# MKimiSH/video-filler

Measured on AMD Instinct MI355X. Metric: netG+netD fwd+bwd images/sec, 128x128 center-mask, higher is better.
Workload: dtype f32

## Files before the change

include/vf_hip.h:

```cpp
#ifndef VF_HIP_H
#define VF_HIP_H
#include <stddef.h>
#include <stdint.h>
#ifdef __cplusplus
extern "C" {
#endif

typedef struct vf_ctx vf_ctx;

enum { VF_ACT_NONE = 0, VF_ACT_LRELU = 1, VF_ACT_RELU = 2, VF_ACT_TANH = 3, VF_ACT_SIGMOID = 4 };

const char* vf_last_error(void);
int vf_version(void);
int vf_ctx_create(vf_ctx** out, int device, void* stream);
int vf_ctx_destroy(vf_ctx* ctx);
int vf_ctx_set_mfma_mode(vf_ctx* ctx, int mode);
int vf_ctx_set_stream(vf_ctx* ctx, void* stream);
int vf_ctx_set_workspace(vf_ctx* ctx, void* ptr, size_t bytes);
size_t vf_workspace_bytes_hint(void);
int vf_stream_synchronize(vf_ctx* ctx);
int vf_malloc(void** out, size_t bytes);
int vf_free(void* ptr);
int vf_memcpy_h2d(vf_ctx* ctx, void* dst, const void* src, size_t bytes);
int vf_memcpy_d2h(vf_ctx* ctx, void* dst, const void* src, size_t bytes);
// ... 154 lines not shown
                   int32_t* status, int32_t* rounds);

int vf_channel_copy(vf_ctx* ctx, const float* src, int Csrc, int c_src, float* dst, int Cdst, int c_dst, int Ccopy,
                    int64_t npix);
int vf_noise_fill(vf_ctx* ctx, float* out, int64_t n, uint64_t seed, const int32_t* counter_dev, uint64_t counter,
                  int normal);

int vf_wgrad_group_begin(vf_ctx* ctx);
int vf_wgrad_group_end(vf_ctx* ctx);
int vf_wgrad_group_abort(vf_ctx* ctx);
int vf_wgrad_group_count(vf_ctx* ctx, int* count);
int vf_wgrad_group_end_partial(vf_ctx* ctx, int count);

int vf_bias_grad_plan(int64_t P, int C, int* cq, int* rows_per_block, int* gx, int* gy);
int vf_bias_grad_multi(vf_ctx* ctx, const void* desc_dev, int n, int blocks1, int blocks2);

typedef struct vf_comm vf_comm;
#define VF_COMM_ID_BYTES 128
int vf_comm_available(void);
int vf_comm_unique_id(void* id128);
int vf_comm_init(vf_comm** out, const void* id128, int world, int rank);
int vf_comm_world(const vf_comm* c);
int vf_comm_rank(const vf_comm* c);
int vf_comm_allreduce_async(vf_comm* c, vf_ctx* ctx, void* buf, int64_t count, int dtype, int op, int* ticket);
int vf_comm_allreduce_avg_async(vf_comm* c, vf_ctx* ctx, float* buf, int64_t n, int* ticket);
int vf_comm_reduce_scatter_avg_async(vf_comm* c, vf_ctx* ctx, float* buf, int64_t shard_count, int* ticket);
int vf_comm_allgather_async(vf_comm* c, vf_ctx* ctx, float* buf, int64_t shard_count, int* ticket);
int vf_comm_broadcast_async(vf_comm* c, vf_ctx* ctx, float* buf, int64_t count, int root, int* ticket);
int vf_comm_wait(vf_comm* c, vf_ctx* ctx, int ticket);
int vf_comm_allreduce_inline(vf_comm* c, vf_ctx* ctx, void* buf, int64_t count, int dtype, int op);
// ... 78 lines not shown
```

video-filler_amd/_lib.py:

```python
import ctypes as C
import os
import re

_HERE = os.path.dirname(os.path.abspath(__file__))
_HEADER = os.path.join(_HERE, "..", "include", "vf_hip.h")

vp, f32, i32, i64, f64, sz, u64 = C.c_void_p, C.c_float, C.c_int, C.c_int64, C.c_double, C.c_size_t, C.c_uint64

SIGNATURES = {
    "vf_last_error": (C.c_char_p, []),
    "vf_version": (i32, []),
    "vf_ctx_create": (i32, [C.POINTER(vp), i32, vp]),
    "vf_ctx_destroy": (i32, [vp]),
    "vf_ctx_set_mfma_mode": (i32, [vp, i32]),
    "vf_ctx_set_stream": (i32, [vp, vp]),
    "vf_ctx_set_workspace": (i32, [vp, vp, sz]),
    "vf_workspace_bytes_hint": (sz, []),
    "vf_stream_synchronize": (i32, [vp]),
    "vf_malloc": (i32, [C.POINTER(vp), sz]),
    "vf_free": (i32, [vp]),
    "vf_memcpy_h2d": (i32, [vp, vp, vp, sz]),
    "vf_memcpy_d2h": (i32, [vp, vp, vp, sz]),
    "vf_zero": (i32, [vp, vp, sz]),
    "vf_zero_segments": (i32, [vp, vp, vp, vp, i32]),
# ... 31 lines not shown
    "vf_bn_fuse_result": (i32, [vp, C.POINTER(i32)]),
    "vf_bn_train_fwd_pre": (i32, [vp, vp, i32] + [vp] * 9 + [i64, i32, i32, f32, f32, i32, f32, vp]),
    "vf_bn_bwd_pre": (i32, [vp, vp, i32] + [vp] * 9 + [i64, i32, i32, f32, vp]),
    "vf_act_fwd": (i32, [vp, vp, vp, i64, i32, f32]),
    "vf_act_bwd": (i32, [vp, vp, vp, vp, i64, i32, f32]),
    "vf_axpby": (i32, [vp, f32, vp, f32, vp, i64]),
    "vf_cmul": (i32, [vp, vp, vp, i64]),
    "vf_scale_shift": (i32, [vp, vp, f32, f32, i64]),
    "vf_masked_compose": (i32, [vp, vp, vp, vp, vp, i64]),
    "vf_conv2d_bwd_data_act": (i32, [vp, vp, vp, vp, vp, i32, f32, i32, i32, i32, i32, i32, i32, i32, i32]),
    "vf_wgrad_group_begin": (i32, [vp]),
    "vf_wgrad_group_end": (i32, [vp]),
    "vf_wgrad_group_abort": (i32, [vp]),
    "vf_bias_grad_plan": (i32, [i64, i32, vp, vp, vp, vp]),
    "vf_bias_grad_multi": (i32, [vp, vp, i32, i32, i32]),
    "vf_center_prepare": (i32, [vp, vp, vp, vp, vp, i32, i32, i32, i32]),
    "vf_clip_prepare": (i32, [vp, vp, vp, vp, vp, vp, i32, i32, i32, i32, i32, i32, i32, f32, i32, i32, vp, vp]),
    "vf_tiles_gather": (i32, [vp, vp, vp, i32, i32, i32, i32, i32, vp]),
    "vf_tiles_scatter": (i32, [vp, vp, vp, i32, i32, i32, i32, i32, vp]),
    "vf_image_scale": (i32, [vp, vp, i32, vp] + [i32] * 6),
    "vf_image_scale_u8": (i32, [vp, vp, vp] + [i32] * 6),
    "vf_image_hook2d": (i32, [vp, vp, i32, vp] + [i32] * 9),
    "vf_image_whole_frames": (i32, [vp, vp, i32, vp] + [i32] * 8 + [vp, f32]),
    "vf_crop_stats": (i32, [vp, vp, vp] + [i32] * 6 + [vp]),
    "vf_jpeg_inspect": (i32, [vp, sz, i32, vp, C.c_char_p, i32]),
    "vf_jpeg_workspace_bytes": (i32, [vp, vp, i32, i32, C.POINTER(sz), C.POINTER(sz)]),
    "vf_jpeg_decode": (i32, [vp, vp, vp, i32, i32, i32, vp, vp, vp, sz, vp, sz, vp, vp]),
    "vf_channel_copy": (i32, [vp, vp, i32, i32, vp, i32, i32, i32, i64]),
    "vf_noise_fill": (i32, [vp, vp, i64, u64, vp, u64, i32]),
    "vf_bce_fwd": (i32, [vp, vp, f32, i32, vp]),
# ... 131 lines not shown
```

video-filler_amd/backend.py:

```python
import ctypes as C
import os

import numpy as np
import torch

from . import _lib

ACT = {"none": 0, "lrelu": 1, "relu": 2, "tanh": 3, "sigmoid": 4}
COLSUM_DESC = [("g", "<u8"), ("gb", "<u8"), ("part", "<u8"), ("P", "<i8"), ("C", "<i4"), ("cq", "<i4"), ("rows_per_block", "<i4"),
               ("gx", "<i4"), ("gy", "<i4"), ("blk1_off", "<i4"), ("blk2_off", "<i4"), ("beta", "<f4")]
WPLANES_DESC = [("w", "<u8"), ("nat", "<u8"), ("tr", "<u8"), ("d0", "<i4"), ("d1", "<i4"), ("gx", "<i4"), ("gz", "<i4"),
                ("blk_off", "<i4"), ("pad", "<i4")]
MFMA_MODES = {"f32": 0, "bf16": 1, "f32_3xbf16": 3}
DEFAULT_MFMA_MODE = "f32_3xbf16"


_COMM_DTYPE = {torch.float32: 0, torch.float64: 1}
_COMM_OP = {"sum": 0, "avg": 1, "max": 2, "min": 3}


class _Range:
    def __init__(self, lib, name):
        self.lib, self.name = lib, name.encode()

# ... 391 lines not shown
    def wgrad_group_abort(self):
        self._c("vf_wgrad_group_abort")

    def wgrad_group_count(self):
        n = C.c_int(0)
        self._c("vf_wgrad_group_count", C.byref(n))
        return n.value

    def wgrad_group_end_partial(self, count):
        self._c("vf_wgrad_group_end_partial", int(count))

    def bias_grad_multi(self, items):
        import numpy as np
        if not items:
            return
        key = tuple((g.data_ptr(), gb.data_ptr(), g.numel(), gb.numel(), float(beta)) for g, gb, beta in items)
        cache = self.__dict__.setdefault("_colsum_plans", {})
        plan = cache.get(key)
        if plan is None:
            desc = np.zeros(len(items), dtype=COLSUM_DESC)
            ws = self.workspace.data_ptr()
            off, b1, b2 = 0, 0, 0
            for i, (g, gb, beta) in enumerate(items):
                Cc = gb.numel()
                P = g.numel() // Cc
                assert Cc % 4 == 0 and g.data_ptr() % 16 == 0 and is_nhwc(g)
                geo = [C.c_int() for _ in range(4)]
                _lib.check(self.lib.vf_bias_grad_plan(P, Cc, *[C.byref(v) for v in geo]))
                cq, rpb, gx, gy = [v.value for v in geo]
                desc[i] = (g.data_ptr(), gb.data_ptr(), ws + off, P, Cc, cq, rpb, gx, gy, b1, b2, beta)
                off += (gx * Cc * 8 + 255) // 256 * 256
                b1 += gx * gy
                b2 += (Cc + 3) // 4
            assert off <= self.workspace.numel(), "workspace too small for the bias-gradient partials"
            dev = torch.from_numpy(desc.view(np.uint8).copy()).to(self.device)
            plan = (dev, len(items), b1, b2)
            cache[key] = plan
        dev, n, b1, b2 = plan
        self._c("vf_bias_grad_multi", _ptr(dev), n, b1, b2)

    def conv2d_bwd_weight(self, x, gy, gw, gb, k, stride, pad, beta, x_planes=None, gy_planes=None):
        B, Cin, H, W = x.shape
        if x_planes is not None and gy_planes is not None:
            self._c("vf_conv2d_bwd_weight_planes", _ptr(x), _ptr(gy), _ptr(x_planes), _ptr(gy_planes), _ptr(gw), _ptr(gb), B, H, W,
                    Cin, gw.shape[0], k, stride, pad, beta)
            return
        self._c("vf_conv2d_bwd_weight", _ptr(x), _ptr(gy), _ptr(gw), _ptr(gb), B, H, W, Cin, gw.shape[0], k, stride,
                pad, beta)

    def deconv2d_fwd(self, x, w, bias, y, k, stride, pad, act="none", slope=0.0):
        B, Cin, H, W = x.shape
        self._c("vf_deconv2d_fwd", _ptr(x), _ptr(w), _ptr(bias), _ptr(y), B, H, W, Cin, w.shape[1], k, stride, pad,
                ACT[act], slope)

# ... 405 lines not shown
```

video-filler_amd/csrc/vf_bn.hip:

```cpp
#include <algorithm>

#include "vf_common.h"

typedef float f32x4 __attribute__((ext_vector_type(4)));
typedef unsigned int u32x2 __attribute__((ext_vector_type(2)));

__device__ __forceinline__ unsigned bn_rne16(float v) {
  const unsigned u = __float_as_uint(v);
  return (u + 0x7FFFu + ((u >> 16) & 1u)) >> 16;
}
__device__ __forceinline__ void bn_store_planes(unsigned short* __restrict__ planes, int64_t pstride, int64_t i, f32x4 v, int npl) {
  if (npl == 1) {
    u32x2 o;
    o[0] = bn_rne16(v[0]) | (bn_rne16(v[1]) << 16);
    o[1] = bn_rne16(v[2]) | (bn_rne16(v[3]) << 16);
    *(u32x2*)(planes + i) = o;
    return;
  }
  float r0 = v[0], r1 = v[1], r2 = v[2], r3 = v[3];
#pragma unroll
  for (int q = 0; q < 3; ++q) {
    const unsigned u0 = __float_as_uint(r0), u1 = __float_as_uint(r1), u2 = __float_as_uint(r2), u3 = __float_as_uint(r3);
    u32x2 o;
    o[0] = __builtin_amdgcn_perm(u1, u0, 0x07060302u);
// ... 665 lines not shown
                       2 * C, sums, (float*)nullptr, (float*)nullptr, (float*)nullptr, (float*)nullptr, 0.0, 0.f, 0.f, (float*)nullptr,
                       0.f, 1);
    VF_LAUNCH_CHECK();
  }
  return bn_bwd_apply_groups(ctx, x, nullptr, g_masked, gx, ggamma, gbeta, gamma, save_mean, save_invstd, sums, npix_per_group,
                             npix_per_group, C, groups, VF_ACT_NONE, 0.f, pbeta, gx_planes);
}

VF_API int vf_bias_grad_plan(int64_t P, int C, int* cq, int* rows_per_block, int* gx, int* gy) {
  VF_REQUIRE(P > 0 && C > 0 && C % 4 == 0, "vf_bias_grad_plan: C must be a positive multiple of 4 (got %d)", C);
  const BnGeom g = bn_geom(P, C, bn_stat_blocks(P, C, 32768));
  *cq = g.cq; *rows_per_block = g.rows_per_block; *gx = g.gx; *gy = g.gy;
  return 0;
}
VF_API int vf_bias_grad_multi(vf_ctx* ctx, const void* desc_dev, int n, int blocks1, int blocks2) {
  VF_REQUIRE(desc_dev != nullptr && n > 0 && blocks1 > 0 && blocks2 > 0, "vf_bias_grad_multi: empty plan");
  VfProf prof(ctx, "bias_grad_multi", 0.0, 0.0);
  hipLaunchKernelGGL(k_colsum4_multi, dim3(blocks1), dim3(256), 0, ctx->stream, (const VfColsumDesc*)desc_dev, n);
  VF_LAUNCH_CHECK();
  hipLaunchKernelGGL(k_reduce_bias_multi, dim3(blocks2), dim3(256), 0, ctx->stream, (const VfColsumDesc*)desc_dev, n);
  VF_LAUNCH_CHECK();
  return 0;
}
```

video-filler_amd/csrc/vf_common.h:

```cpp
#pragma once
#include <hip/hip_runtime.h>
#include <hip/hip_ext.h>

#include <cstdarg>
#include <cstdint>
#include <cstdio>
#include <cstring>

#include "../../include/vf_hip.h"

#define VF_API extern "C" __attribute__((visibility("default")))

struct VfBnSt {
  int mode;
  const float* vec;
  const float* x;
  double* part;
  int rows_per_group;
  int tiles_per_group;
  int zpar;
};

struct vf_ctx {
  int device;
// ... 4 lines not shown
  int mfma_bf16;
  int wg_active;
  void* wg_rec;
  VfBnSt bnf;
  const float* bnf_yact;
  int bnf_act;
  float bnf_slope;
  int bnf_groups, bnf_rows_cap;
  int bnf_result_rows;
  unsigned* act_bits_out;
  int act_bits_written;
  const unsigned* dmask_bits;
  const float* dot_act_y;
  int dot_act;
  float dot_act_slope;
};
void vf_internal_wg_free(vf_ctx* ctx);

unsigned vf_error_seq();
struct VfOneShotScope {
  vf_ctx* c;
  unsigned seq;
  explicit VfOneShotScope(vf_ctx* ctx) : c(ctx), seq(vf_error_seq()) {}
  ~VfOneShotScope() {
    if (!c || vf_error_seq() == seq) return;
    c->bnf.mode = 0;
    c->bnf_result_rows = 0;
    c->act_bits_out = nullptr;
    c->act_bits_written = 0;
    c->dmask_bits = nullptr;
    c->dot_act_y = nullptr;
  }
};

static inline char* vf_ws_ptr(vf_ctx* c) { return (char*)c->ws + c->ws_front; }
static inline size_t vf_ws_avail(vf_ctx* c) { return c->ws_bytes > c->ws_front ? c->ws_bytes - c->ws_front : 0; }

void vf_set_error(const char* fmt, ...);

#define VF_CHECK_HIP(expr)                                                              \
  do {                                                                                  \
    hipError_t _e = (expr);                                                             \
    if (_e != hipSuccess) {                                                             \
      vf_set_error("%s:%d: %s failed: %s", __FILE__, __LINE__, #expr, hipGetErrorString(_e)); \
      return 1;                                                                         \
    }                                                                                   \
// ... 133 lines not shown
```

video-filler_amd/csrc/vf_conv.hip:

```cpp
#include <algorithm>
#include <vector>
#include <cstdlib>

#include "vf_common.h"

typedef float f32x16 __attribute__((ext_vector_type(16)));
typedef float f32x4 __attribute__((ext_vector_type(4)));
typedef unsigned int u32x4 __attribute__((ext_vector_type(4)));
typedef __bf16 bf16x8 __attribute__((ext_vector_type(8)));
typedef __bf16 bf16x4 __attribute__((ext_vector_type(4)));

#define VF_OOB 0x80000000u
__device__ __forceinline__ __amdgpu_buffer_rsrc_t vf_rsrc(const void* p, unsigned bytes) {
  return __builtin_amdgcn_make_buffer_rsrc(const_cast<void*>(p), 0, bytes, 0x00020000);
}
__device__ __forceinline__ f32x4 vf_bload4(__amdgpu_buffer_rsrc_t r, unsigned byte_off) {
  return __builtin_bit_cast(f32x4, __builtin_amdgcn_raw_buffer_load_b128(r, byte_off, 0, 0));
}
__device__ __forceinline__ float vf_bload1(__amdgpu_buffer_rsrc_t r, unsigned byte_off) {
  return __builtin_bit_cast(float, __builtin_amdgcn_raw_buffer_load_b32(r, byte_off, 0, 0));
}

template <int LD>
__device__ __forceinline__ bf16x8 vf_tr_frag(const __bf16* tile, int col0, int k0, int lane) {
// ... 764 lines not shown
}

struct WGrad {
  const float* U;
  const float* V;
  float* dW;
  float* slab;
  unsigned u_bytes, v_bytes;
  int P, lgMh, lgMw;
  int Nu, Cv, Hv, Wv;
  int stride, pad;
  int ntaps;
  int gx, gy, gz;
  int ksplit, nk;
  float beta;
};

template <int BM, bool VU, bool VV, int BF = 0>
__device__ __forceinline__ void wgrad_body(const WGrad& p, const int block_id) {
  constexpr int BN = 128, BK = BF ? 32 : 16;
  constexpr int LDU = BM + 4, LDV = BN + 4;
  constexpr int WN = BM == 128 ? 64 : 32;
  constexpr int NT = WN / 32;
  constexpr int WAVES_N = BN / WN;
  constexpr int U_CH = (BK * BM / 4) / 256;
  constexpr int V_CH = (BK * BN / 4) / 256;
  constexpr int U_SZ = BK * LDU, V_SZ = BK * LDV;
  constexpr int LDMU = BM + 32, LDMV = BN + 32;
  constexpr int UH_SZ = BK * LDMU, VH_SZ = BK * LDMV;
  constexpr int NP = BF > 0 ? BF : 1;
// ... 16 lines not shown
  int v_dy[4], v_dx[4], v_c[4];
  bool v_okc[4];
#pragma unroll
  for (int j = 0; j < 4; ++j) {
    const int col = j0 + 4 * cq + j;
    v_okc[j] = col < Ncols;
    const int tap = v_okc[j] ? col / p.Cv : 0;
    v_c[j] = v_okc[j] ? col - tap * p.Cv : 0;
    v_dy[j] = (tap >> 2) - p.pad;
    v_dx[j] = (tap & 3) - p.pad;
  }
  const int uq = tid % (BM / 4), ukk = tid / (BM / 4);
  const int un = n0 + 4 * uq;

  f32x4 ru[U_CH], rv[V_CH];
  const __amdgpu_buffer_rsrc_t rsU = vf_rsrc(p.U, p.u_bytes), rsV = vf_rsrc(p.V, p.v_bytes);

  auto load_piece = [&](int kt, int pc, bool live) {
    if (pc < U_CH) {
      const int i = pc;
      const int pp = kt * BK + ukk + i * (1024 / BM);
      const bool okp = live && pp < p.P;
      if constexpr (VU) {
        ru[i] = vf_bload4(rsU, (okp && un < p.Nu) ? 4u * (unsigned)(pp * p.Nu + un) : VF_OOB);
      } else {
        f32x4 v;
#pragma unroll
        for (int j = 0; j < 4; ++j) {
          v[j] = vf_bload1(rsU, (okp && un + j < p.Nu) ? 4u * (unsigned)(pp * p.Nu + un + j) : VF_OOB);
        }
// ... 10 lines not shown
        const bool ok = okp && v_okc[0] && (unsigned)iy < (unsigned)p.Hv && (unsigned)ix < (unsigned)p.Wv;
        rv[i] = vf_bload4(rsV, ok ? 4u * (unsigned)(boff + (iy * p.Wv + ix) * p.Cv + v_c[0]) : VF_OOB);
      } else {
        f32x4 v;
#pragma unroll
        for (int j = 0; j < 4; ++j) {
          const int iy = my * p.stride + v_dy[j], ix = mx * p.stride + v_dx[j];
          const bool ok = okp && v_okc[j] && (unsigned)iy < (unsigned)p.Hv && (unsigned)ix < (unsigned)p.Wv;
          v[j] = vf_bload1(rsV, ok ? 4u * (unsigned)(boff + (iy * p.Wv + ix) * p.Cv + v_c[j]) : VF_OOB);
        }
        rv[i] = v;
      }
    }
  };
  auto store_piece = [&](int buf, int pc) {
    if constexpr (BF) {
      __bf16* base = (__bf16*)smem + buf * (NP * PL_SZ);
      f32x4 v;
      int off;
      if (pc < U_CH) {
        v = ru[pc];
        off = (ukk + pc * (1024 / BM)) * LDMU + 4 * uq;
      } else {
        const int i = pc - U_CH;
        v = rv[i];
        off = UH_SZ + ((tid >> 5) + 8 * i) * LDMV + 4 * cq;
      }
      if constexpr (NP == 3) {
        const VfPlanes3 s3 = vf_split3(v);
#pragma unroll
// ... 102 lines not shown
      for (int j = 0; j < 4; ++j)
#pragma unroll
        for (int mt = 0; mt < 2; ++mt)
#pragma unroll
          for (int nt = 0; nt < NT; ++nt) {
            acc[mt][nt] = __builtin_amdgcn_mfma_f32_32x32x2f32(fa[ss][mt][j], fb[ss][nt][j], acc[mt][nt], 0, 0, 0);
            const int slot = ss * NMF + (j * 2 + mt) * NT + nt;
            if (slot < NPC) load_piece(kt + 1, slot, more);
            if (slot >= SLOTS - NPC) store_piece(buf ^ 1, slot - (SLOTS - NPC));
            __builtin_amdgcn_sched_barrier(0);
          }
    }
    __syncthreads();
  }

  }
  const int64_t total = (int64_t)p.Nu * Ncols;
  float* out = p.ksplit > 1 ? p.slab + (int64_t)ks * total : p.dW;
#pragma unroll
  for (int mt = 0; mt < 2; ++mt)
#pragma unroll
    for (int r = 0; r < 16; ++r) {
      const int n = n0 + wm + mt * 32 + (r & 3) + 8 * (r >> 2) + 4 * lh;
      if (n >= p.Nu) continue;
#pragma unroll
      for (int nt = 0; nt < NT; ++nt) {
        const int col = j0 + wn + nt * 32 + lr;
        if (col < Ncols) {
          const int64_t idx = (int64_t)n * Ncols + col;
          float v = acc[mt][nt][r];
// ... 673 lines not shown
    const int rc = wg_flush(ctx);
    R->ws_used = used;
    return rc;
  }
  std::vector<WgRec> rest(R->recs.begin() + count, R->recs.end());
  R->recs.resize((size_t)count);
  const size_t used = R->ws_used;
  const int rc = wg_flush(ctx);
  R->recs = rest;
  R->ws_used = used;
  return rc;
}

int vf_internal_wgrad_smallk(vf_ctx* ctx, const float* U, const float* V, float* dW, int K, int Nu, int Ncols, float beta);
static int wgrad(vf_ctx* ctx, const float* U, const float* V, float* dW, int B, int Hl, int Wl, int Nu, int Hv, int Wv,
                 int Cv, int stride, int pad, float beta, int ntaps = 16, const void* Up = nullptr, const void* Vp = nullptr) {
  if (Hl == 1 && Wl == 1 && Hv == 4 && Wv == 4 && stride == 1 && pad == 0 && ntaps == 16) {
    const int rc = vf_internal_wgrad_smallk(ctx, U, V, dW, B, Nu, 16 * Cv, beta);
    if (rc >= 0) return rc;
  }
  WGrad g;
  memset(&g, 0, sizeof(g));
  g.U = U; g.V = V; g.dW = dW;
  g.P = B * Hl * Wl;
  g.lgMh = vf_ilog2(Hl); g.lgMw = vf_ilog2(Wl);
  g.Nu = Nu; g.Cv = Cv; g.Hv = Hv; g.Wv = Wv;
  g.stride = stride; g.pad = pad;
  g.ntaps = ntaps;
  g.nk = (int)vf_cdiv(g.P, ctx->mfma_bf16 ? 32 : 16);
  VF_REQUIRE((int64_t)g.P * Nu < ((int64_t)1 << 29) && (int64_t)B * Hv * Wv * Cv < ((int64_t)1 << 29),
             "operand exceeds the 2 GiB buffer-descriptor range");
// ... 7 lines not shown
  const int64_t blocks = (int64_t)gx * gy;
  const int64_t total = (int64_t)Nu * ntaps * Cv;
  int ksplit = 1;
  const bool use_pw = Up && Vp && (ctx->mfma_bf16 == 3 || ctx->mfma_bf16 == 1) && ntaps == 16 && stride == 2 && pad == 1 && Nu % 128 == 0 &&
                      Cv % 64 == 0 && g.P % 32 == 0 && (int64_t)g.P * Nu * 6 < ((int64_t)1 << 31) &&
                      (int64_t)B * Hv * Wv * Cv * 6 < ((int64_t)1 << 31) && total % 4 == 0;
  const int wg_blocks = use_pw ? 256 : 512;
  if (blocks < wg_blocks * 3 / 4 && g.nk >= 16) {
    ksplit = (int)std::min<int64_t>(g.nk / 8, vf_cdiv(wg_blocks, blocks));
    while (ksplit > 1 && (size_t)ksplit * total * sizeof(float) > vf_ws_avail(ctx)) --ksplit;
    if (ksplit < 1) ksplit = 1;
    const int steps = (int)vf_cdiv(g.nk, ksplit);
    ksplit = (int)vf_cdiv(g.nk, steps);
  }
  g.ksplit = ksplit;
  g.slab = ksplit > 1 ? (float*)vf_ws_ptr(ctx) : nullptr;
  g.gx = gx; g.gy = gy; g.gz = ksplit;
  dim3 grid((unsigned)gx * gy * ksplit), block(256);
  const bool own_group = use_pw && !ctx->wg_active;
  if (own_group) {
    if (!ctx->wg_rec) ctx->wg_rec = new WgRecorder();
    ctx->wg_active = 1;
  }
  if (ctx->wg_active && (use_pw || (vecU && vecV && (ksplit == 1 || total % 4 == 0)))) {
    WgRecorder* R = (WgRecorder*)ctx->wg_rec;
    const size_t need = ksplit > 1 ? (((size_t)ksplit * total * sizeof(float) + 255) & ~(size_t)255) : 0;
    if (R->ws_used + need > vf_ws_avail(ctx)) {
      if (int rc = wg_flush(ctx)) return rc;
      R->ws_used = 0;
    }
// ... 70 lines not shown
    if (BM == 128) {
      if (bf == 3) VF_WG(128, 3); else if (bf) VF_WG(128, 1); else VF_WG(128, 0);
    } else {
      if (bf == 3) VF_WG(64, 3); else if (bf) VF_WG(64, 1); else VF_WG(64, 0);
    }
#undef VF_WG
  }
  VF_LAUNCH_CHECK();
  if (ksplit > 1) {
    VfProf prof(ctx, "slab_reduce_wgrad", 0.0, 4.0 * (double)total * (ksplit + 1));
    return launch_slab_reduce(ctx, g.slab, dW, nullptr, total, 1, ksplit, VF_ACT_NONE, 0.f, beta);
  }
  return 0;
}

int vf_internal_colsum(vf_ctx* ctx, const float* g, float* gb, int64_t P, int C, float beta);
static int bias_grad(vf_ctx* ctx, const float* g, float* gb, int64_t P, int C, float beta) {
  return vf_internal_colsum(ctx, g, gb, P, C, beta);
}

int vf_internal_gconv_fwd(vf_ctx* ctx, const float* x, const float* w, const float* bias, float* y, int B, int H, int W, int Cin,
                          int Cout, int k, int stride, int pad, int act, float slope);
int vf_internal_gconv_bwd_data(vf_ctx* ctx, const float* gy, const float* w, float* gx, int B, int H, int W, int Cin, int Cout,
                               int k, int stride, int pad);
int vf_internal_gconv_bwd_weight(vf_ctx* ctx, const float* x, const float* gy, float* gw, float* gb, int B, int H, int W, int Cin,
                                 int Cout, int k, int stride, int pad, float beta);
static bool main_net_shape(int H, int W, int k, int stride, int pad) {
  return k == 4 && ((stride == 2 && pad == 1) || (stride == 1 && pad == 0 && H == 4 && W == 4)) && vf_is_pow2(H) && vf_is_pow2(W);
}

// ... 48 lines not shown
static int conv2d_bwd_weight_impl(vf_ctx* ctx, const float* x, const float* gy, const void* x_planes, const void* gy_planes,
                                  float* gw, float* gb, int B, int H, int W, int Cin, int Cout, int k, int stride, int pad, float beta);
VF_API int vf_conv2d_bwd_weight(vf_ctx* ctx, const float* x, const float* gy, float* gw, float* gb, int B, int H, int W,
                                int Cin, int Cout, int k, int stride, int pad, float beta) {
  VfOneShotScope one_shot(ctx);
  return conv2d_bwd_weight_impl(ctx, x, gy, nullptr, nullptr, gw, gb, B, H, W, Cin, Cout, k, stride, pad, beta);
}
VF_API int vf_conv2d_bwd_weight_planes(vf_ctx* ctx, const float* x, const float* gy, const void* x_planes, const void* gy_planes,
                                       float* gw, float* gb, int B, int H, int W, int Cin, int Cout, int k, int stride, int pad,
                                       float beta) {
  VfOneShotScope one_shot(ctx);
  return conv2d_bwd_weight_impl(ctx, x, gy, x_planes, gy_planes, gw, gb, B, H, W, Cin, Cout, k, stride, pad, beta);
}
static int conv2d_bwd_weight_impl(vf_ctx* ctx, const float* x, const float* gy, const void* x_planes, const void* gy_planes,
                                  float* gw, float* gb, int B, int H, int W, int Cin, int Cout, int k, int stride, int pad, float beta) {
  if (!main_net_shape(H, W, k, stride, pad))
    return vf_internal_gconv_bwd_weight(ctx, x, gy, gw, gb, B, H, W, Cin, Cout, k, stride, pad, beta);
  if (int rc = check_conv_args(B, H, W, Cin, Cout, k, stride, pad)) return rc;
  const int Ho = (H + 2 * pad - 4) / stride + 1, Wo = (W + 2 * pad - 4) / stride + 1;
  if (Cout == 1 && stride == 1 && H == 4 && W == 4) {
    const float* ya = ctx->dot_act_y;
    ctx->dot_act_y = nullptr;
    hipLaunchKernelGGL(k_dot_bwd_weight, dim3((int)vf_cdiv(16 * Cin, 64)), dim3(512), 0, ctx->stream, x, gy, gw, gb, B,
                       16 * Cin, beta, ya, ctx->dot_act, ctx->dot_act_slope);
    VF_LAUNCH_CHECK();
    return 0;
  }
  if (int rc = wgrad(ctx, gy, x, gw, B, Ho, Wo, Cout, H, W, Cin, stride, pad, beta, 16, gy_planes, x_planes)) return rc;
  if (gb) return bias_grad(ctx, gy, gb, (int64_t)B * Ho * Wo, Cout, beta);
  return 0;
}

VF_API int vf_deconv2d_fwd(vf_ctx* ctx, const float* x, const float* w, const float* bias, float* y, int B, int H, int W,
                           int Cin, int Cout, int k, int stride, int pad, int act, float slope) {
  VfOneShotScope one_shot(ctx);
  VF_REQUIRE(k == 4 && ((stride == 2 && pad == 1) || (stride == 1 && pad == 0)), "unsupported full-conv shape");
  VF_REQUIRE(vf_is_pow2(H) && vf_is_pow2(W), "spatial sizes must be powers of two");
  return conv_like_bwd(ctx, x, w, bias, y, B, H, W, Cin, Cout, stride, pad, act, slope);
}

VF_API int vf_deconv2d_bwd_data(vf_ctx* ctx, const float* gy, const float* w, float* gx, int B, int H, int W, int Cin,
                                int Cout, int k, int stride, int pad) {
  VfOneShotScope one_shot(ctx);
  VF_REQUIRE(k == 4 && ((stride == 2 && pad == 1) || (stride == 1 && pad == 0)), "unsupported full-conv shape");
  const int Ho = (H - 1) * stride - 2 * pad + 4, Wo = (W - 1) * stride - 2 * pad + 4;
  VF_REQUIRE(vf_is_pow2(H) && vf_is_pow2(W), "spatial sizes must be powers of two");
  return conv_like_fwd(ctx, gy, w, nullptr, gx, B, Ho, Wo, Cout, Cin, stride, pad, VF_ACT_NONE, 0.f);
}

static int deconv2d_bwd_weight_impl(vf_ctx* ctx, const float* x, const float* gy, const void* x_planes, const void* gy_planes,
                                    float* gw, float* gb, int B, int H, int W, int Cin, int Cout, int k, int stride, int pad,
                                    float beta) {
  VF_REQUIRE(k == 4 && ((stride == 2 && pad == 1) || (stride == 1 && pad == 0)), "unsupported full-conv shape");
  VF_REQUIRE(vf_is_pow2(H) && vf_is_pow2(W), "spatial sizes must be powers of two");
  const int Ho = (H - 1) * stride - 2 * pad + 4, Wo = (W - 1) * stride - 2 * pad + 4;
  if (int rc = wgrad(ctx, x, gy, gw, B, H, W, Cin, Ho, Wo, Cout, stride, pad, beta, 16, x_planes, gy_planes)) return rc;
  if (gb) return bias_grad(ctx, gy, gb, (int64_t)B * Ho * Wo, Cout, beta);
  return 0;
}
VF_API int vf_deconv2d_bwd_weight(vf_ctx* ctx, const float* x, const float* gy, float* gw, float* gb, int B, int H, int W,
                                  int Cin, int Cout, int k, int stride, int pad, float beta) {
  VfOneShotScope one_shot(ctx);
  return deconv2d_bwd_weight_impl(ctx, x, gy, nullptr, nullptr, gw, gb, B, H, W, Cin, Cout, k, stride, pad, beta);
}
VF_API int vf_deconv2d_bwd_weight_planes(vf_ctx* ctx, const float* x, const float* gy, const void* x_planes, const void* gy_planes,
                                         float* gw, float* gb, int B, int H, int W, int Cin, int Cout, int k, int stride, int pad,
                                         float beta) {
// ... 4 lines not shown
```

video-filler_amd/csrc/vf_net.hip:

```cpp
#include <algorithm>
#include <cstdlib>
#include <cstring>
#include <map>
#include <string>
#include <vector>

#include "vf_common.h"

int vf_internal_colsum(vf_ctx* ctx, const float* g, float* gb, int64_t P, int C, float beta);

namespace {

double g_gate_gflop = getenv("VF_PCONV_MIN_GFLOP") ? atof(getenv("VF_PCONV_MIN_GFLOP")) : 3.0;
int g_gate_rows = getenv("VF_PCONV_MIN_ROWS") ? atoi(getenv("VF_PCONV_MIN_ROWS")) : 1024;
const bool g_no_pconv = getenv("VF_NO_PCONV") != nullptr;
const bool g_no_bn_fuse = getenv("VF_NO_BN_FUSE") != nullptr;
const bool g_pwgrad = !(getenv("VF_PWGRAD") && strcmp(getenv("VF_PWGRAD"), "1") != 0);

struct VfColsumDescH {
  const float* g;
  float* gb;
  double* part;
  int64_t P;
  int C, cq, rows_per_block, gx, gy;
// ... 10 lines not shown
static_assert(sizeof(VfWpDescH) == 48, "descriptor layout is shared with vf_pgemm.hip");

struct Layer {
  vf_layer_desc d;
  int C = 0, H = 0, W = 0;
  int Co = 0, Ho = 0, Wo = 0;
  int64_t w_off = -1, b_off = -1, w_n = 0, b_n = 0;
  float* y = nullptr;
  float* y_own = nullptr;
  float* gx = nullptr;
  float* gtmp = nullptr;
  float *rm = nullptr, *rv = nullptr, *sm = nullptr, *si = nullptr;
  double* sums = nullptr;
  double* part = nullptr;
  int part_rows_cap = 0;
  void* xp = nullptr;
  void* gp = nullptr;
  void* yp = nullptr;
  void* bgp = nullptr;
  unsigned* ybits = nullptr;
  bool bits_live = false;
  const void* out_planes = nullptr;
  const void* grad_planes = nullptr;
  void *wp_nat = nullptr, *wp_tr = nullptr;
  bool wp_live = false;
  int wp_mode = 0;
  const float* x_seen = nullptr;
  const void* xp_seen = nullptr;
  const float* g_seen = nullptr;
  const void* gp_seen = nullptr;
// ... 256 lines not shown
    return rc;
  }
  l.g_seen = nullptr;
  if (in_act != VF_ACT_NONE)
    return vf_conv2d_bwd_data_act(ctx, go, w, l.gx, x, in_act, in_slope, Bn, l.H, l.W, l.C, l.Co, l.d.k, l.d.stride, l.d.pad);
  return full ? vf_deconv2d_bwd_data(ctx, go, w, l.gx, Bn, l.H, l.W, l.C, l.Co, l.d.k, l.d.stride, l.d.pad)
              : vf_conv2d_bwd_data(ctx, go, w, l.gx, Bn, l.H, l.W, l.C, l.Co, l.d.k, l.d.stride, l.d.pad);
}

struct Deferred {
  const float* g;
  float* gb;
  int64_t P;
  int C;
  float beta;
};

int conv_acc(vf_net* n, Layer& l, const float* x, const float* go, int Bn, std::vector<Deferred>* deferred) {
  vf_ctx* ctx = n->ctx;
  const bool full = is_full(l);
  float* gw = n->grads + l.w_off;
  float* gb = n->grads + l.b_off;
  const float beta = l.fresh ? 0.f : 1.f;
  l.fresh = false;
  if (deferred && l.Co % 4 == 0 && ((uintptr_t)go & 15) == 0) {
    deferred->push_back(Deferred{go, gb, (int64_t)Bn * l.Ho * l.Wo, l.Co, beta});
    gb = nullptr;
  }
  VF_REQUIRE(!(n->fused_adam && l.fa && l.fa_k > 0 && beta != 0.f),
             "fused Adam: a second backward pass accumulates onto a weight gradient that was never written (one backward per zeroGradParameters)");
  if (n->fused_adam && l.fa && beta == 0.f) {
    l.fa_u = full ? x : go;
    l.fa_v = full ? go : x;
    l.fa_k = Bn;
    l.g_seen = nullptr;
    l.gp_seen = nullptr;
    if (!gb) return 0;
    return vf_internal_colsum(ctx, go, gb, (int64_t)Bn * l.Ho * l.Wo, l.Co, beta);
  }
  l.fa_k = 0;
  const bool planes = g_pwgrad && !g_no_pconv && l.x_seen == x && l.xp_seen && l.g_seen == go && l.gp_seen;
  const void *xp = l.xp_seen, *gp = l.gp_seen;
  l.g_seen = nullptr;
  l.gp_seen = nullptr;
  if (planes)
    return full ? vf_deconv2d_bwd_weight_planes(ctx, x, go, xp, gp, gw, gb, Bn, l.H, l.W, l.C, l.Co, l.d.k, l.d.stride, l.d.pad, beta)
                : vf_conv2d_bwd_weight_planes(ctx, x, go, xp, gp, gw, gb, Bn, l.H, l.W, l.C, l.Co, l.d.k, l.d.stride, l.d.pad, beta);
  return full ? vf_deconv2d_bwd_weight(ctx, x, go, gw, gb, Bn, l.H, l.W, l.C, l.Co, l.d.k, l.d.stride, l.d.pad, beta)
              : vf_conv2d_bwd_weight(ctx, x, go, gw, gb, Bn, l.H, l.W, l.C, l.Co, l.d.k, l.d.stride, l.d.pad, beta);
}

int bn_backward(vf_net* n, Layer& l, const float* x, const float* gy, int Bn, bool want_gx, bool want_gp, int act, float slope,
                const float* y_act, int gsel, int pre_rows, bool want_planes) {
  vf_ctx* ctx = n->ctx;
  VF_REQUIRE(n->train, "vf_net_backward: BatchNorm backward in evaluate mode is not part of the path");
  const float* gamma = n->params + l.w_off;
  float* gg = want_gp ? n->grads + l.w_off : nullptr;
  float* gbt = want_gp ? n->grads + l.b_off : nullptr;
  float* gx = want_gx ? l.gx : nullptr;
  float pbeta = 1.f;
  if (want_gp) {
    pbeta = l.fresh ? 0.f : 1.f;
    l.fresh = false;
  }
// ... 31 lines not shown
}

int bias_grad_flush(vf_net* n, const std::vector<Deferred>& items) {
  if (items.empty()) return 0;
  std::string key((const char*)items.data(), items.size() * sizeof(Deferred));
  auto it = n->colsum_plans.find(key);
  if (it == n->colsum_plans.end()) {
    std::vector<VfColsumDescH> desc(items.size());
    char* ws = vf_ws_ptr(n->ctx);
    size_t off = 0;
    int b1 = 0, b2 = 0;
    for (size_t i = 0; i < items.size(); ++i) {
      const Deferred& d = items[i];
      int cq, rpb, gx, gy;
      if (int rc = vf_bias_grad_plan(d.P, d.C, &cq, &rpb, &gx, &gy)) return rc;
      desc[i] = VfColsumDescH{d.g, d.gb, (double*)(ws + off), d.P, d.C, cq, rpb, gx, gy, b1, b2, d.beta};
      off += ((size_t)gx * d.C * 8 + 255) / 256 * 256;
      b1 += gx * gy;
      b2 += (d.C + 3) / 4;
    }
    VF_REQUIRE(off <= vf_ws_avail(n->ctx), "vf_net: workspace too small for the bias-gradient partials");
    void* dev = nullptr;
    if (int rc = net_alloc(n->owned, &dev, desc.size() * sizeof(VfColsumDescH))) return rc;
    VF_CHECK_HIP(hipMemcpy(dev, desc.data(), desc.size() * sizeof(VfColsumDescH), hipMemcpyHostToDevice));
    it = n->colsum_plans.emplace(key, std::make_pair(dev, std::vector<int>{(int)items.size(), b1, b2})).first;
  }
  const std::vector<int>& g = it->second.second;
  return vf_bias_grad_multi(n->ctx, it->second.first, g[0], g[1], g[2]);
}

int net_walk_back(vf_net* n, const float* x_in, const float* gy, const float** gx_out, bool want_gp, bool need_input_grad, int hi,
                  int lo, int gi, int G, int defer_cut = -1) {
  vf_ctx* ctx = n->ctx;
// ... 177 lines not shown
        VF_REQUIRE(l.d.nout == c, "vf_net: BatchNorm layer %d has %d channels, gets %d", (int)i, l.d.nout, c);
        break;
      default:
        break;
    }
    VF_REQUIRE(l.Ho > 0 && l.Wo > 0, "vf_net: layer %d has an empty output", (int)i);
    c = l.Co; h = l.Ho; w = l.Wo;
    l.y = l.y_own = l.gx = l.gtmp = nullptr;
    l.xp = l.gp = l.yp = l.bgp = nullptr;
    l.ybits = nullptr;
    l.bits_live = false;
    l.out_planes = l.grad_planes = nullptr;
    l.x_seen = l.g_seen = nullptr;
    l.xp_seen = l.gp_seen = nullptr;
    l.part = nullptr;
    l.sm = l.si = nullptr;
    l.sums = nullptr;
  }
  n->gcap = std::max(n->groups, 2);
  for (size_t i = 0; i < n->L.size(); ++i) {
    Layer& l = n->L[i];
    const size_t in_e = (size_t)B * l.H * l.W * l.C, out_e = (size_t)B * l.Ho * l.Wo * l.Co;
    const bool own_out = is_conv(l) || l.d.kind == VF_L_BN || (l.d.kind == VF_L_ACT && !l.absorbed);
    if (own_out) {
      if (int rc = net_alloc(n->act_owned, (void**)&l.y_own, sizeof(float) * out_e)) return rc;
      l.y = l.y_own;
    }
    if (is_conv(l) || l.d.kind == VF_L_BN || (l.d.kind == VF_L_ACT && !l.absorbed))
      if (int rc = net_alloc(n->act_owned, (void**)&l.gx, sizeof(float) * in_e)) return rc;
    if (l.d.kind == VF_L_BN) {
// ... 587 lines not shown
```

video-filler_amd/nn.py:

```python
import torch

from .backend import bump_param_version, get_backend, is_nhwc, param_version, to_nhwc


class DeviceScalar:

    def __init__(self, fn):
        self._fn = fn

    @staticmethod
    def of(t):
        return DeviceScalar(lambda: float(t.item()))

    def __float__(self):
        return float(self._fn())

    def _bin(self, other, op):
        a, b = self, other
        return DeviceScalar(lambda: op(float(a), float(b)))

    def __add__(self, o):
        return self._bin(o, lambda x, y: x + y)

    __radd__ = __add__
# ... 154 lines not shown
            if self._is_full:
                B.pconv_gather(gp, wp, None, gx, Bn, Ho, Wo, Co, self.nInputPlane)
            elif in_act is not None:
                B.pconv_scatter(gp, wp, None, gx, Bn, Ho, Wo, Co, self.nInputPlane, dmask=input, dact=in_act[0], dslope=in_act[1])
            else:
                B.pconv_scatter(gp, wp, None, gx, Bn, Ho, Wo, Co, self.nInputPlane)
            return gx
        self._g_planes = None
        if in_act is not None:
            B.conv2d_bwd_data_act(to_nhwc(gradOutput), self.weight, gx, input, in_act[0], in_act[1], self.kH, self.dH, self.padH)
            return gx
        fn = B.deconv2d_bwd_data if self._is_full else B.conv2d_bwd_data
        fn(to_nhwc(gradOutput), self.weight, gx, self.kH, self.dH, self.padH)
        return gx

    def accGradParameters(self, input, gradOutput, scale=1, defer_bias=None, use_planes=True):
        assert scale == 1, "the reference always uses scale = 1"
        beta = 0.0 if self._fresh else 1.0
        self._fresh = False
        fn = get_backend().deconv2d_bwd_weight if self._is_full else get_backend().conv2d_bwd_weight
        go = to_nhwc(gradOutput)
        gb = self.gradBias
        if defer_bias is not None and self.nOutputPlane % 4 == 0 and go.data_ptr() % 16 == 0:
            defer_bias.append((go, self.gradBias, beta))
            gb = None
        x = to_nhwc(input)
        xs, gs = getattr(self, "_x_planes", None), getattr(self, "_g_planes", None)
        self._g_planes = None
        if (use_planes and _PWGRAD and not _NO_PCONV and xs is not None and gs is not None and xs[0] == x.data_ptr()
                and xs[1] == tuple(x.shape) and gs[0] == go.data_ptr() and gs[1] == tuple(go.shape)):
            fn(x, go, self.gradWeight, gb, self.kH, self.dH, self.padH, beta, xs[2], gs[2])
        else:
            fn(x, go, self.gradWeight, gb, self.kH, self.dH, self.padH, beta)

    def parameters(self):
        return [self.weight, self.bias], [self.gradWeight, self.gradBias]


class SpatialFullConvolution(SpatialConvolution):
    _type = "nn.SpatialFullConvolution"
    _is_full = True


class SpatialBatchNormalization(Module):
    _type = "nn.SpatialBatchNormalization"

    def __init__(self, nOutput, eps=1e-5, momentum=0.1, affine=True):
        super().__init__()
# ... 636 lines not shown
                            return out
                    elif isinstance(m, SpatialConvolution):
                        upd = lambda: m.updateGradInput(x, g, in_act, gbuf, g_planes=g_pl, managed=managed)
                    elif group is not None and isinstance(m, _Act):
                        upd = lambda: m.updateGradInput(x, g, mout)
                    else:
                        upd = lambda: m.updateGradInput(x, g)
                    if want_gp and self.side is not None and m.parameters():
                        with self.side.on():
                            self._acc(m, x, g, deferred, use_planes=False)
                        used_side = True
                        gin = upd() if want_gx else None
                    else:
                        gin = upd() if want_gx else None
                        if want_gp:
                            self._acc(m, x, g, deferred)
                    g = gin
                    g_pl = None
                    act_done = in_act is not None
                    bn_pre, pre[0] = pre[0], 0
                    continue
                act_done = False
        except BaseException:
            if grouped:
                Sequential._group_open = False
                B.wgrad_group_abort()
            raise
        if cut_wg is not None:
            if grouped:
                B.wgrad_group_end_partial(cut_wg)
            if deferred:
# ... 3 lines not shown
        else:
            if grouped:
                Sequential._group_open = False
                B.wgrad_group_end()
            if deferred:
                B.bias_grad_multi(deferred)
        if used_side:
            self.side.join()
        self._act_done_at = lo if act_done else -1
        self._bn_pre_at = (lo, bn_pre) if (bn_pre and lo > 0) else None
        if lo == 0:
            self.gradInput = g
        return g

    @staticmethod
    def _acc(m, x, g, deferred, use_planes=True):
        if isinstance(m, SpatialConvolution):
            m.accGradParameters(x, g, 1, deferred, use_planes)
        else:
            m.accGradParameters(x, g, 1)

    def refresh_weight_planes(self):
        B = get_backend()
        if self._flat is not None:
            self._wp_version = param_version(self._flat[0])
        if _NO_PCONV or getattr(B, "mfma_mode", None) not in _PLANES_MODES or not hasattr(B, "weight_planes_multi"):
            return
        mods = [m for m in self.leaves() if isinstance(m, SpatialConvolution) and getattr(m, "_wp_live", False)
                and m._wp_src == m.weight.data_ptr() and getattr(m, "_wp_mode", None) == B.mfma_mode]
        if not mods:
            return
        key = tuple(m.weight.data_ptr() for m in mods)
        if self._wp_plan is None or self._wp_plan[3] != key:
# ... 272 lines not shown
```

Baseline: 22830.

## Fuse bias-gradient column sums into the weight-gradient GEMM operand loads

The weight-gradient kernel now accumulates the gradOutput operand it already loads into per-thread sums and writes per-ksplit partial column sums in double into a per-layer buffer. The deferred bias-gradient reduction then skips its own colsum pass over gradOutput for those layers and only runs the final reduce over the provided partial rows. This removes a full extra read of the output gradient per conv layer, at the cost of extra smem reduction work and registers in the wgrad kernel and more plumbing through context state.

```diff
diff --git a/include/vf_hip.h b/include/vf_hip.h
--- a/include/vf_hip.h
+++ b/include/vf_hip.h
@@ -192,6 +192,8 @@
 
 int vf_bias_grad_plan(int64_t P, int C, int* cq, int* rows_per_block, int* gx, int* gy);
 int vf_bias_grad_multi(vf_ctx* ctx, const void* desc_dev, int n, int blocks1, int blocks2);
+int vf_bias_part_next(vf_ctx* ctx, double* part, int rows_cap);
+int vf_bias_part_result(vf_ctx* ctx, int* rows, int* run);
 
 typedef struct vf_comm vf_comm;
 #define VF_COMM_ID_BYTES 128
diff --git a/video-filler_amd/_lib.py b/video-filler_amd/_lib.py
--- a/video-filler_amd/_lib.py
+++ b/video-filler_amd/_lib.py
@@ -69,6 +69,8 @@
     "vf_wgrad_group_abort": (i32, [vp]),
     "vf_bias_grad_plan": (i32, [i64, i32, vp, vp, vp, vp]),
     "vf_bias_grad_multi": (i32, [vp, vp, i32, i32, i32]),
+    "vf_bias_part_next": (i32, [vp, vp, i32]),
+    "vf_bias_part_result": (i32, [vp, C.POINTER(i32), C.POINTER(i32)]),
     "vf_center_prepare": (i32, [vp, vp, vp, vp, vp, i32, i32, i32, i32]),
     "vf_clip_prepare": (i32, [vp, vp, vp, vp, vp, vp, i32, i32, i32, i32, i32, i32, i32, f32, i32, i32, vp, vp]),
     "vf_tiles_gather": (i32, [vp, vp, vp, i32, i32, i32, i32, i32, vp]),
diff --git a/video-filler_amd/backend.py b/video-filler_amd/backend.py
--- a/video-filler_amd/backend.py
+++ b/video-filler_amd/backend.py
@@ -429,23 +429,28 @@
         import numpy as np
         if not items:
             return
-        key = tuple((g.data_ptr(), gb.data_ptr(), g.numel(), gb.numel(), float(beta)) for g, gb, beta in items)
+        items = [tuple(it) + (None, 0) if len(it) == 3 else tuple(it) for it in items]
+        key = tuple((g.data_ptr(), gb.data_ptr(), g.numel(), gb.numel(), float(beta), 0 if part is None else part.data_ptr(), rows)
+                    for g, gb, beta, part, rows in items)
         cache = self.__dict__.setdefault("_colsum_plans", {})
         plan = cache.get(key)
         if plan is None:
             desc = np.zeros(len(items), dtype=COLSUM_DESC)
             ws = self.workspace.data_ptr()
             off, b1, b2 = 0, 0, 0
-            for i, (g, gb, beta) in enumerate(items):
+            for i, (g, gb, beta, part, rows) in enumerate(items):
                 Cc = gb.numel()
                 P = g.numel() // Cc
                 assert Cc % 4 == 0 and g.data_ptr() % 16 == 0 and is_nhwc(g)
                 geo = [C.c_int() for _ in range(4)]
                 _lib.check(self.lib.vf_bias_grad_plan(P, Cc, *[C.byref(v) for v in geo]))
                 cq, rpb, gx, gy = [v.value for v in geo]
-                desc[i] = (g.data_ptr(), gb.data_ptr(), ws + off, P, Cc, cq, rpb, gx, gy, b1, b2, beta)
-                off += (gx * Cc * 8 + 255) // 256 * 256
-                b1 += gx * gy
+                if rows > 0:
+                    desc[i] = (g.data_ptr(), gb.data_ptr(), part.data_ptr(), P, Cc, cq, rpb, rows, 0, b1, b2, beta)
+                else:
+                    desc[i] = (g.data_ptr(), gb.data_ptr(), ws + off, P, Cc, cq, rpb, gx, gy, b1, b2, beta)
+                    off += (gx * Cc * 8 + 255) // 256 * 256
+                    b1 += gx * gy
                 b2 += (Cc + 3) // 4
             assert off <= self.workspace.numel(), "workspace too small for the bias-gradient partials"
             dev = torch.from_numpy(desc.view(np.uint8).copy()).to(self.device)
@@ -453,6 +458,16 @@
             cache[key] = plan
         dev, n, b1, b2 = plan
         self._c("vf_bias_grad_multi", _ptr(dev), n, b1, b2)
+
+    BIAS_PART_ROWS = 512
+
+    def bias_part_next(self, part):
+        self._c("vf_bias_part_next", _ptr(part), part.shape[0])
+
+    def bias_part_result(self):
+        rows, run = C.c_int(0), C.c_int(0)
+        self._c("vf_bias_part_result", C.byref(rows), C.byref(run))
+        return rows.value, run.value
 
     def conv2d_bwd_weight(self, x, gy, gw, gb, k, stride, pad, beta, x_planes=None, gy_planes=None):
         B, Cin, H, W = x.shape
diff --git a/video-filler_amd/csrc/vf_bn.hip b/video-filler_amd/csrc/vf_bn.hip
--- a/video-filler_amd/csrc/vf_bn.hip
+++ b/video-filler_amd/csrc/vf_bn.hip
@@ -703,10 +703,12 @@
   return 0;
 }
 VF_API int vf_bias_grad_multi(vf_ctx* ctx, const void* desc_dev, int n, int blocks1, int blocks2) {
-  VF_REQUIRE(desc_dev != nullptr && n > 0 && blocks1 > 0 && blocks2 > 0, "vf_bias_grad_multi: empty plan");
+  VF_REQUIRE(desc_dev != nullptr && n > 0 && blocks1 >= 0 && blocks2 > 0, "vf_bias_grad_multi: empty plan");
   VfProf prof(ctx, "bias_grad_multi", 0.0, 0.0);
-  hipLaunchKernelGGL(k_colsum4_multi, dim3(blocks1), dim3(256), 0, ctx->stream, (const VfColsumDesc*)desc_dev, n);
-  VF_LAUNCH_CHECK();
+  if (blocks1 > 0) {
+    hipLaunchKernelGGL(k_colsum4_multi, dim3(blocks1), dim3(256), 0, ctx->stream, (const VfColsumDesc*)desc_dev, n);
+    VF_LAUNCH_CHECK();
+  }
   hipLaunchKernelGGL(k_reduce_bias_multi, dim3(blocks2), dim3(256), 0, ctx->stream, (const VfColsumDesc*)desc_dev, n);
   VF_LAUNCH_CHECK();
   return 0;
diff --git a/video-filler_amd/csrc/vf_common.h b/video-filler_amd/csrc/vf_common.h
--- a/video-filler_amd/csrc/vf_common.h
+++ b/video-filler_amd/csrc/vf_common.h
@@ -42,6 +42,8 @@
   const float* dot_act_y;
   int dot_act;
   float dot_act_slope;
+  double* bp_part;
+  int bp_cap, bp_rows, bp_run;
 };
 void vf_internal_wg_free(vf_ctx* ctx);
 
@@ -58,6 +60,8 @@
     c->act_bits_written = 0;
     c->dmask_bits = nullptr;
     c->dot_act_y = nullptr;
+    c->bp_part = nullptr;
+    c->bp_cap = c->bp_rows = c->bp_run = 0;
   }
 };
 
diff --git a/video-filler_amd/csrc/vf_conv.hip b/video-filler_amd/csrc/vf_conv.hip
--- a/video-filler_amd/csrc/vf_conv.hip
+++ b/video-filler_amd/csrc/vf_conv.hip
@@ -802,6 +802,7 @@
   int gx, gy, gz;
   int ksplit, nk;
   float beta;
+  double* bpart;
 };
 
 template <int BM, bool VU, bool VV, int BF = 0>
@@ -848,6 +849,7 @@
   const int un = n0 + 4 * uq;
 
   f32x4 ru[U_CH], rv[V_CH];
+  f32x4 usum = {0.f, 0.f, 0.f, 0.f};
   const __amdgpu_buffer_rsrc_t rsU = vf_rsrc(p.U, p.u_bytes), rsV = vf_rsrc(p.V, p.v_bytes);
 
   auto load_piece = [&](int kt, int pc, bool live) {
@@ -888,6 +890,7 @@
     }
   };
   auto store_piece = [&](int buf, int pc) {
+    if (pc < U_CH) usum += ru[pc];
     if constexpr (BF) {
       __bf16* base = (__bf16*)smem + buf * (NP * PL_SZ);
       f32x4 v;
@@ -1020,6 +1023,23 @@
     __syncthreads();
   }
 
+  }
+  if (p.bpart != nullptr && j0 == 0) {
+    constexpr int UROWS = 1024 / BM;
+    f32x4* red = (f32x4*)smem;
+    red[tid] = usum;
+    __syncthreads();
+    if (ukk == 0) {
+      double a[4] = {0, 0, 0, 0};
+      for (int j = 0; j < UROWS; ++j) {
+        const f32x4 u = red[j * (BM / 4) + uq];
+#pragma unroll
+        for (int e = 0; e < 4; ++e) a[e] += (double)u[e];
+      }
+#pragma unroll
+      for (int e = 0; e < 4; ++e)
+        if (un + e < p.Nu) p.bpart[(int64_t)ks * p.Nu + un + e] = a[e];
+    }
   }
   const int64_t total = (int64_t)p.Nu * Ncols;
   float* out = p.ksplit > 1 ? p.slab + (int64_t)ks * total : p.dW;
@@ -1723,7 +1743,8 @@
 
 int vf_internal_wgrad_smallk(vf_ctx* ctx, const float* U, const float* V, float* dW, int K, int Nu, int Ncols, float beta);
 static int wgrad(vf_ctx* ctx, const float* U, const float* V, float* dW, int B, int Hl, int Wl, int Nu, int Hv, int Wv,
-                 int Cv, int stride, int pad, float beta, int ntaps = 16, const void* Up = nullptr, const void* Vp = nullptr) {
+                 int Cv, int stride, int pad, float beta, int ntaps = 16, const void* Up = nullptr, const void* Vp = nullptr,
+                 double* bpart = nullptr, int bcap = 0) {
   if (Hl == 1 && Wl == 1 && Hv == 4 && Wv == 4 && stride == 1 && pad == 0 && ntaps == 16) {
     const int rc = vf_internal_wgrad_smallk(ctx, U, V, dW, B, Nu, 16 * Cv, beta);
     if (rc >= 0) return rc;
@@ -1761,6 +1782,11 @@
     ksplit = (int)vf_cdiv(g.nk, steps);
   }
   g.ksplit = ksplit;
+  if (bpart && !use_pw && !(Hl == 1 && Wl == 1) && ntaps == 16 && ksplit <= bcap) {
+    g.bpart = bpart;
+    ctx->bp_rows = ksplit;
+    ctx->bp_run = (int)vf_cdiv(g.nk, ksplit) * ((ctx->mfma_bf16 ? 32 : 16) * BM / 1024);
+  }
   g.slab = ksplit > 1 ? (float*)vf_ws_ptr(ctx) : nullptr;
   g.gx = gx; g.gy = gy; g.gz = ksplit;
   dim3 grid((unsigned)gx * gy * ksplit), block(256);
@@ -1861,6 +1887,29 @@
   return 0;
 }
 
+VF_API int vf_bias_part_next(vf_ctx* ctx, double* part, int rows_cap) {
+  VF_REQUIRE(ctx && part && rows_cap > 0, "vf_bias_part_next: bad arguments");
+  ctx->bp_part = part;
+  ctx->bp_cap = rows_cap;
+  ctx->bp_rows = ctx->bp_run = 0;
+  return 0;
+}
+VF_API int vf_bias_part_result(vf_ctx* ctx, int* rows, int* run) {
+  VF_REQUIRE(ctx && rows, "vf_bias_part_result: NULL");
+  *rows = ctx->bp_rows;
+  if (run) *run = ctx->bp_run;
+  ctx->bp_part = nullptr;
+  ctx->bp_cap = ctx->bp_rows = ctx->bp_run = 0;
+  return 0;
+}
+static double* take_bias_part(vf_ctx* ctx, int* cap) {
+  double* p = ctx->bp_part;
+  *cap = ctx->bp_cap;
+  ctx->bp_part = nullptr;
+  ctx->bp_cap = ctx->bp_rows = ctx->bp_run = 0;
+  return p;
+}
+
 int vf_internal_colsum(vf_ctx* ctx, const float* g, float* gb, int64_t P, int C, float beta);
 static int bias_grad(vf_ctx* ctx, const float* g, float* gb, int64_t P, int C, float beta) {
   return vf_internal_colsum(ctx, g, gb, P, C, beta);
@@ -1939,6 +1988,8 @@
 }
 static int conv2d_bwd_weight_impl(vf_ctx* ctx, const float* x, const float* gy, const void* x_planes, const void* gy_planes,
                                   float* gw, float* gb, int B, int H, int W, int Cin, int Cout, int k, int stride, int pad, float beta) {
+  int bcap = 0;
+  double* bpart = take_bias_part(ctx, &bcap);
   if (!main_net_shape(H, W, k, stride, pad))
     return vf_internal_gconv_bwd_weight(ctx, x, gy, gw, gb, B, H, W, Cin, Cout, k, stride, pad, beta);
   if (int rc = check_conv_args(B, H, W, Cin, Cout, k, stride, pad)) return rc;
@@ -1951,7 +2002,7 @@
     VF_LAUNCH_CHECK();
     return 0;
   }
-  if (int rc = wgrad(ctx, gy, x, gw, B, Ho, Wo, Cout, H, W, Cin, stride, pad, beta, 16, gy_planes, x_planes)) return rc;
+  if (int rc = wgrad(ctx, gy, x, gw, B, Ho, Wo, Cout, H, W, Cin, stride, pad, beta, 16, gy_planes, x_planes, bpart, bcap)) return rc;
   if (gb) return bias_grad(ctx, gy, gb, (int64_t)B * Ho * Wo, Cout, beta);
   return 0;
 }
@@ -1976,6 +2027,8 @@
 static int deconv2d_bwd_weight_impl(vf_ctx* ctx, const float* x, const float* gy, const void* x_planes, const void* gy_planes,
                                     float* gw, float* gb, int B, int H, int W, int Cin, int Cout, int k, int stride, int pad,
                                     float beta) {
+  int bcap = 0;
+  (void)take_bias_part(ctx, &bcap);
   VF_REQUIRE(k == 4 && ((stride == 2 && pad == 1) || (stride == 1 && pad == 0)), "unsupported full-conv shape");
   VF_REQUIRE(vf_is_pow2(H) && vf_is_pow2(W), "spatial sizes must be powers of two");
   const int Ho = (H - 1) * stride - 2 * pad + 4, Wo = (W - 1) * stride - 2 * pad + 4;
diff --git a/video-filler_amd/csrc/vf_net.hip b/video-filler_amd/csrc/vf_net.hip
--- a/video-filler_amd/csrc/vf_net.hip
+++ b/video-filler_amd/csrc/vf_net.hip
@@ -48,6 +48,7 @@
   double* sums = nullptr;
   double* part = nullptr;
   int part_rows_cap = 0;
+  double* bpart = nullptr;
   void* xp = nullptr;
   void* gp = nullptr;
   void* yp = nullptr;
@@ -334,7 +335,11 @@
   int64_t P;
   int C;
   float beta;
+  double* part;
+  int rows, pad_;
 };
+static_assert(sizeof(Deferred) == 48, "Deferred is compared and stored as bytes");
+constexpr int BIAS_PART_ROWS = 512;
 
 int conv_acc(vf_net* n, Layer& l, const float* x, const float* go, int Bn, std::vector<Deferred>* deferred) {
   vf_ctx* ctx = n->ctx;
@@ -343,9 +348,11 @@
   float* gb = n->grads + l.b_off;
   const float beta = l.fresh ? 0.f : 1.f;
   l.fresh = false;
+  bool bias_deferred = false;
   if (deferred && l.Co % 4 == 0 && ((uintptr_t)go & 15) == 0) {
-    deferred->push_back(Deferred{go, gb, (int64_t)Bn * l.Ho * l.Wo, l.Co, beta});
+    deferred->push_back(Deferred{go, gb, (int64_t)Bn * l.Ho * l.Wo, l.Co, beta, nullptr, 0, 0});
     gb = nullptr;
+    bias_deferred = true;
   }
   VF_REQUIRE(!(n->fused_adam && l.fa && l.fa_k > 0 && beta != 0.f),
              "fused Adam: a second backward pass accumulates onto a weight gradient that was never written (one backward per zeroGradParameters)");
@@ -363,11 +370,28 @@
   const void *xp = l.xp_seen, *gp = l.gp_seen;
   l.g_seen = nullptr;
   l.gp_seen = nullptr;
+  const bool arm = bias_deferred && !full;
+  if (arm) {
+    if (!l.bpart)
+      if (int rc = net_alloc(n->act_owned, (void**)&l.bpart, sizeof(double) * (size_t)BIAS_PART_ROWS * l.Co)) return rc;
+    if (int rc = vf_bias_part_next(ctx, l.bpart, BIAS_PART_ROWS)) return rc;
+  }
+  int rc;
   if (planes)
-    return full ? vf_deconv2d_bwd_weight_planes(ctx, x, go, xp, gp, gw, gb, Bn, l.H, l.W, l.C, l.Co, l.d.k, l.d.stride, l.d.pad, beta)
-                : vf_conv2d_bwd_weight_planes(ctx, x, go, xp, gp, gw, gb, Bn, l.H, l.W, l.C, l.Co, l.d.k, l.d.stride, l.d.pad, beta);
-  return full ? vf_deconv2d_bwd_weight(ctx, x, go, gw, gb, Bn, l.H, l.W, l.C, l.Co, l.d.k, l.d.stride, l.d.pad, beta)
+    rc = full ? vf_deconv2d_bwd_weight_planes(ctx, x, go, xp, gp, gw, gb, Bn, l.H, l.W, l.C, l.Co, l.d.k, l.d.stride, l.d.pad, beta)
+              : vf_conv2d_bwd_weight_planes(ctx, x, go, xp, gp, gw, gb, Bn, l.H, l.W, l.C, l.Co, l.d.k, l.d.stride, l.d.pad, beta);
+  else
+    rc = full ? vf_deconv2d_bwd_weight(ctx, x, go, gw, gb, Bn, l.H, l.W, l.C, l.Co, l.d.k, l.d.stride, l.d.pad, beta)
               : vf_conv2d_bwd_weight(ctx, x, go, gw, gb, Bn, l.H, l.W, l.C, l.Co, l.d.k, l.d.stride, l.d.pad, beta);
+  if (arm && !rc) {
+    int rows = 0;
+    if ((rc = vf_bias_part_result(ctx, &rows, nullptr))) return rc;
+    if (rows > 0) {
+      deferred->back().part = l.bpart;
+      deferred->back().rows = rows;
+    }
+  }
+  return rc;
 }
 
 int bn_backward(vf_net* n, Layer& l, const float* x, const float* gy, int Bn, bool want_gx, bool want_gp, int act, float slope,
@@ -429,9 +453,13 @@
       const Deferred& d = items[i];
       int cq, rpb, gx, gy;
       if (int rc = vf_bias_grad_plan(d.P, d.C, &cq, &rpb, &gx, &gy)) return rc;
-      desc[i] = VfColsumDescH{d.g, d.gb, (double*)(ws + off), d.P, d.C, cq, rpb, gx, gy, b1, b2, d.beta};
-      off += ((size_t)gx * d.C * 8 + 255) / 256 * 256;
-      b1 += gx * gy;
+      if (d.rows > 0) {
+        desc[i] = VfColsumDescH{d.g, d.gb, d.part, d.P, d.C, cq, rpb, d.rows, 0, b1, b2, d.beta};
+      } else {
+        desc[i] = VfColsumDescH{d.g, d.gb, (double*)(ws + off), d.P, d.C, cq, rpb, gx, gy, b1, b2, d.beta};
+        off += ((size_t)gx * d.C * 8 + 255) / 256 * 256;
+        b1 += gx * gy;
+      }
       b2 += (d.C + 3) / 4;
     }
     VF_REQUIRE(off <= vf_ws_avail(n->ctx), "vf_net: workspace too small for the bias-gradient partials");
@@ -639,6 +667,7 @@
     l.x_seen = l.g_seen = nullptr;
     l.xp_seen = l.gp_seen = nullptr;
     l.part = nullptr;
+    l.bpart = nullptr;
     l.sm = l.si = nullptr;
     l.sums = nullptr;
   }
diff --git a/video-filler_amd/nn.py b/video-filler_amd/nn.py
--- a/video-filler_amd/nn.py
+++ b/video-filler_amd/nn.py
@@ -192,16 +192,24 @@
         fn(to_nhwc(gradOutput), self.weight, gx, self.kH, self.dH, self.padH)
         return gx
 
-    def accGradParameters(self, input, gradOutput, scale=1, defer_bias=None, use_planes=True):
+    def accGradParameters(self, input, gradOutput, scale=1, defer_bias=None, use_planes=True, bias_part=False):
         assert scale == 1, "the reference always uses scale = 1"
         beta = 0.0 if self._fresh else 1.0
         self._fresh = False
         fn = get_backend().deconv2d_bwd_weight if self._is_full else get_backend().conv2d_bwd_weight
         go = to_nhwc(gradOutput)
         gb = self.gradBias
+        B = get_backend()
+        arm = False
         if defer_bias is not None and self.nOutputPlane % 4 == 0 and go.data_ptr() % 16 == 0:
             defer_bias.append((go, self.gradBias, beta))
             gb = None
+            arm = bias_part and not self._is_full and hasattr(B, "bias_part_next")
+        if arm:
+            part = getattr(self, "_bias_part", None)
+            if part is None:
+                part = self._bias_part = torch.empty((B.BIAS_PART_ROWS, self.nOutputPlane), dtype=torch.float64, device=go.device)
+            B.bias_part_next(part)
         x = to_nhwc(input)
         xs, gs = getattr(self, "_x_planes", None), getattr(self, "_g_planes", None)
         self._g_planes = None
@@ -210,6 +218,10 @@
             fn(x, go, self.gradWeight, gb, self.kH, self.dH, self.padH, beta, xs[2], gs[2])
         else:
             fn(x, go, self.gradWeight, gb, self.kH, self.dH, self.padH, beta)
+        if arm:
+            rows, _ = B.bias_part_result()
+            if rows > 0:
+                defer_bias[-1] = (go, self.gradBias, beta, part, rows)
 
     def parameters(self):
         return [self.weight, self.bias], [self.gradWeight, self.gradBias]
@@ -876,7 +888,7 @@
                     else:
                         gin = upd() if want_gx else None
                         if want_gp:
-                            self._acc(m, x, g, deferred)
+                            self._acc(m, x, g, deferred, bias_part=grouped or not Sequential._group_open)
                     g = gin
                     g_pl = None
                     act_done = in_act is not None
@@ -910,9 +922,9 @@
         return g
 
     @staticmethod
-    def _acc(m, x, g, deferred, use_planes=True):
+    def _acc(m, x, g, deferred, use_planes=True, bias_part=False):
         if isinstance(m, SpatialConvolution):
-            m.accGradParameters(x, g, 1, deferred, use_planes)
+            m.accGradParameters(x, g, 1, deferred, use_planes, bias_part)
         else:
             m.accGradParameters(x, g, 1)
 
```

After: 23000, median of 6. About the same (+0.7%).
